# Chengyuann/AutoStyle-TTS

Hardware: AMD Instinct MI355X
Metric: synthesized audio sec/wall-sec (RTF^-1) + style-kNN QPS, IEMOCAP test batch (higher is better)
Workload: dtype f16; 1 GPU; BASELINE configs[1]: batch=8 utterances/GPU, kNN Q=8 x N=1000 x D=6144 k=3, synthesis Tt=32 Tp=150 Ts=250 (fixed-length decode, EOS ignored) -> 430 mel frames -> 110080 samples @ 22050 Hz; CosyVoice-300M shapes, random-init weights; parallelism=dp1 (model + bank replicated, utterances sharded, all-gather of style ids only)

## Files before the change

### autostyle-tts_amd/csrc/ops_audio.hip

```cpp
#include "common.h"
#include "toplist.h"
#include "xlane.h"

namespace astts {

static constexpr double kTwoPi = 6.283185307179586476925286766559;

__global__ __launch_bounds__(256) void f0_prefix(const float* __restrict__ f0, double* __restrict__ pre, int tm) {
    __shared__ double carry;
    __shared__ double buf[256];
    const int b = blockIdx.x, tid = threadIdx.x;
    if (tid == 0) carry = 0.0;
    __syncthreads();
    for (int base = 0; base < tm; base += 256) {
        const int i = base + tid;
        const double v = i < tm ? (double)f0[(int64_t)b * tm + i] : 0.0;
        buf[tid] = v;
        __syncthreads();
        for (int off = 1; off < 256; off <<= 1) {
            const double add = tid >= off ? buf[tid - off] : 0.0;
            __syncthreads();
            buf[tid] += add;
            __syncthreads();
        }
        if (i < tm) pre[(int64_t)b * tm + i] = carry + buf[tid] - v;
        __syncthreads();
        if (tid == 255) carry += buf[255];
        __syncthreads();
    }
}

struct NsfArgs {
    const float* f0;
    const double* pre;
    const float* phase0;
    const float* noise;
    const float* lin_w;
    const float* lin_b;
    float* out;
    int b, tm, up, nh;
    float sr, sine_amp, noise_std, voiced_thr;
};

__global__ __launch_bounds__(256) void nsf_source(NsfArgs a) {
    const int64_t L = (int64_t)a.tm * a.up;
    const int64_t total = (int64_t)a.b * L;
    for (int64_t i = (int64_t)blockIdx.x * 256 + threadIdx.x; i < total; i += (int64_t)gridDim.x * 256) {
        const int bb = (int)(i / L);
        const int64_t s = i - (int64_t)bb * L;
        const int f = (int)(s / a.up);
        const int r = (int)(s - (int64_t)f * a.up);
        const float f0 = a.f0[(int64_t)bb * a.tm + f];
        const double cum = (a.pre[(int64_t)bb * a.tm + f] * (double)a.up + (double)(r + 1) * (double)f0) / (double)a.sr;
        const float uv = f0 > a.voiced_thr ? 1.0f : 0.0f;
        const float namp = uv * a.noise_std + (1.0f - uv) * a.sine_amp / 3.0f;
        float acc = a.lin_b[0];
        for (int hI = 0; hI < a.nh; ++hI) {
            double ph = cum * (double)(hI + 1);
            ph -= floor(ph);
            const float theta = (float)(kTwoPi * ph);
            const float sine = a.sine_amp * sinf(theta + a.phase0[bb * a.nh + hI]);
            const float v = sine * uv + namp * a.noise[i * a.nh + hI];
            acc += a.lin_w[hI] * v;
        }
        a.out[i] = tanhf(acc);
    }
}

__device__ __forceinline__ float hann16(int n) {
    return 0.5f - 0.5f * cosf((float)(kTwoPi / 16.0) * (float)n);
}

__global__ __launch_bounds__(256) void stft16(const float* __restrict__ x, float* __restrict__ y, int b, int64_t Lmax, int64_t F,
                                              const int* __restrict__ lens) {
    const int64_t total = (int64_t)b * F;
    for (int64_t i = (int64_t)blockIdx.x * 256 + threadIdx.x; i < total; i += (int64_t)gridDim.x * 256) {
        const int bb = (int)(i / F);
        const int64_t f = i - (int64_t)bb * F;
        const float* xb = x + (int64_t)bb * Lmax;
        const int64_t L = lens ? min((int64_t)lens[bb], Lmax) : Lmax;
        float* o = y + i * 18;
        if (f > L / 4) {
#pragma unroll
            for (int k = 0; k < 18; ++k) o[k] = 0.0f;
            continue;
        }
        float w[16];
#pragma unroll
        for (int n = 0; n < 16; ++n) {
            int64_t s = 4 * f - 8 + n;
            if (s < 0) s = -s;
            if (s >= L) s = 2 * (L - 1) - s;
            w[n] = hann16(n) * xb[s];
        }
#pragma unroll
        for (int k = 0; k < 9; ++k) {
            float re = 0.0f, im = 0.0f;
#pragma unroll
            for (int n = 0; n < 16; ++n) {
                const int ph = (k * n) & 15;
                const float cs = cosf((float)(kTwoPi / 16.0) * (float)ph);
                const float sn = sinf((float)(kTwoPi / 16.0) * (float)ph);
                re += w[n] * cs;
                im -= w[n] * sn;
            }
            o[k] = re;
            o[9 + k] = im;
        }
    }
}

__global__ __launch_bounds__(256) void istft16(const float* __restrict__ y, float* __restrict__ wav, int b, int64_t Fmax,
                                               float mag_clip, float audio_limit, const int* __restrict__ frame_lens) {
    const int64_t L = 4 * (Fmax - 1);
    const int64_t total = (int64_t)b * L;
    for (int64_t i = (int64_t)blockIdx.x * 256 + threadIdx.x; i < total; i += (int64_t)gridDim.x * 256) {
        const int bb = (int)(i / L);
        const int64_t t = i - (int64_t)bb * L;
        const int64_t F = frame_lens ? min((int64_t)frame_lens[bb], Fmax) : Fmax;
        if (t >= 4 * (F - 1)) {
            wav[i] = 0.0f;
            continue;
        }
        const int64_t tp = t + 8;
        float num = 0.0f, den = 0.0f;
        const int64_t f_hi = tp / 4;
#pragma unroll
        for (int q = 0; q < 4; ++q) {
            const int64_t f = f_hi - q;
            const int n = (int)(tp - 4 * f);
            if (f < 0 || f >= F) continue;
            const float* fr = y + ((int64_t)bb * Fmax + f) * 18;
            float xs = 0.0f;
#pragma unroll
            for (int k = 0; k < 9; ++k) {
                const float mag = fminf(__expf(fr[k]), mag_clip);
                const float ph = sinf(fr[9 + k]);
                const float re = mag * cosf(ph), im = mag * sinf(ph);
                const int idx = (k * n) & 15;
                const float cs = cosf((float)(kTwoPi / 16.0) * (float)idx);
                const float sn = sinf((float)(kTwoPi / 16.0) * (float)idx);
                const float ck = (k == 0 || k == 8) ? 1.0f : 2.0f;
                xs += ck * (re * cs - ((k == 0 || k == 8) ? 0.0f : im * sn));
            }
            const float wn = hann16(n);
            num += wn * xs * (1.0f / 16.0f);
            den += wn * wn;
        }
        const float v = den > 1e-11f ? num / den : 0.0f;
        wav[i] = fminf(fmaxf(v, -audio_limit), audio_limit);
    }
}

struct SampleArgs {
    const float* logits;
    const int* history;
    const float* u;
    int* out;
    int* hist_w;
    const int* forced;
    int clamp_out;
    const int* eos_min_rows;
    int b, v, hist_len, hist_ld, top_k, win, eos, ignore_eos;
    float top_p, tau_r;
};

static constexpr int RS_NT = 1024;
__global__ __launch_bounds__(RS_NT) void ras_sample(const float* p_logits, const int* p_eos_min_rows, int p_v, int p_hist_len, int p_eos, int p_ignore_eos,
                                                    SampleArgs a_in) {
    __builtin_amdgcn_s_setprio(3);
    SampleArgs a = a_in;
    a.logits = p_logits; a.eos_min_rows = p_eos_min_rows; a.v = p_v; a.hist_len = p_hist_len; a.eos = p_eos; a.ignore_eos = p_ignore_eos;
    extern __shared__ float prob[];
    __shared__ float red_max[RS_NT / 64], red_sum[RS_NT / 64];
    __shared__ float sh_s[RS_NT];
    __shared__ int sh_i[RS_NT];
    __shared__ float s_bcast;
    __shared__ int s_tok;
    __shared__ unsigned hist[3][2048];
    __shared__ int s_sel_bin[3], s_sel_rem[3], s_cnt;
    const int bb = blockIdx.x, tid = threadIdx.x, lane = tid & 63, wid = tid >> 6;
    const float* lg = a.logits + (int64_t)bb * a.v;
    const bool eos_window = a.eos_min_rows ? (a.hist_len < a.eos_min_rows[bb]) : ((a.ignore_eos & 1) != 0);
    const bool reject = eos_window && (a.ignore_eos & 2) != 0;
    const bool mask_eos = eos_window && !reject;
    const int h0 = a.hist_len > a.win ? a.hist_len - a.win : 0;
    const bool win_in_wave = a.hist_len - h0 <= 64;
    float u_first = 0.0f, u_second = 0.0f;
    int hwin = -1;
    if (wid == 0) {
        u_first = a.u[bb * 2];
        u_second = a.u[bb * 2 + 1];
        if (win_in_wave && h0 + lane < a.hist_len) hwin = a.history[(int64_t)bb * a.hist_ld + h0 + lane];
    }
    for (int i = tid; i < 3 * 2048; i += RS_NT) (&hist[0][0])[i] = 0u;
    if (tid == 0) s_cnt = 0;
    if (tid < 16 && ((a.v + 15) & ~15) - 16 + tid >= a.v) prob[((a.v + 15) & ~15) - 16 + tid] = 0.0f;
    float mx = -INFINITY;
    for (int base = 0; base < a.v; base += 8 * RS_NT) {
        float xv[8];
#pragma unroll
        for (int u = 0; u < 8; ++u) xv[u] = lg[min(base + u * RS_NT + tid, a.v - 1)];
#pragma unroll
        for (int u = 0; u < 8; ++u) {
            const int i = base + u * RS_NT + tid;
            if (i < a.v) {
                float x = xv[u];
                if (mask_eos && i == a.eos) x = -INFINITY;
                prob[i] = x;
                mx = fmaxf(mx, x);
            }
        }
    }
    mx = xmax<1>(xmax<2>(xmax<4>(xmax<8>(xmax<16>(xmax<32>(mx))))));
    if (lane == 0) red_max[wid] = mx;
    __syncthreads();
    mx = red_max[0];
#pragma unroll
    for (int w = 1; w < RS_NT / 64; ++w) mx = fmaxf(mx, red_max[w]);
    float sum = 0.0f;
    for (int i = tid; i < a.v; i += RS_NT) {
        const float e = __expf(prob[i] - mx);
        prob[i] = e;
        sum += e;
    }
    sum = wave_sum_desc(sum);
    if (lane == 0) red_sum[wid] = sum;
    __syncthreads();
    float tot = 0.0f;
#pragma unroll
    for (int w = 0; w < RS_NT / 64; ++w) tot += red_sum[w];
    const float inv = 1.0f / tot;
    const int kk = a.top_k < 64 ? a.top_k : 64;
    TopList<float> tl;
    tl.init();
    unsigned prefix = 0u, known = 0u;
    {
        int remaining = kk < a.v ? kk : a.v;
#pragma unroll 1
        for (int pass = 0; pass < 3; ++pass) {
            const int shift = pass == 0 ? 21 : (pass == 1 ? 10 : 0);
            const int bins = pass == 2 ? 1024 : 2048;
            unsigned* h = hist[pass];
            for (int i = tid; i < a.v; i += RS_NT) {
                float pv = prob[i];
                if (pass == 0) {
                    pv *= inv;
                    prob[i] = pv;
                }
                const unsigned key = __float_as_uint(pv);
                if ((key & known) == prefix) atomicAdd(&h[(key >> shift) & (bins - 1)], 1u);
            }
            __syncthreads();
            if (wid == 0) {
                const int per = bins >> 6;
                unsigned hv[32];
#pragma unroll
                for (int j = 0; j < 32; ++j) hv[j] = j < per ? h[lane * per + j] : 0u;
                unsigned local = 0u;
#pragma unroll
                for (int j = 0; j < 32; ++j) local += hv[j];
                unsigned incl = local;
#pragma unroll
                for (int off = 1; off < 64; off <<= 1) {
                    const unsigned tv = __shfl_down(incl, off, 64);
                    if (lane + off < 64) incl += tv;
                }
                const unsigned above = incl - local;
                if (above < (unsigned)remaining && (unsigned)remaining <= incl) {
                    unsigned acc = above;
                    bool done = false;
#pragma unroll
                    for (int j = 31; j >= 0; --j) {
                        if (j < per && !done) {
                            if (acc + hv[j] >= (unsigned)remaining) {
                                s_sel_bin[pass] = lane * per + j;
                                s_sel_rem[pass] = remaining - (int)acc;
                                done = true;
                            } else {
                                acc += hv[j];
                            }
                        }
                    }
                }
            }
            __syncthreads();
            prefix |= (unsigned)s_sel_bin[pass] << shift;
            known |= (unsigned)(bins - 1) << shift;
            remaining = s_sel_rem[pass];
        }
        for (int i = tid; i < a.v; i += RS_NT) {
            if (__float_as_uint(prob[i]) >= prefix) {
                const int pos = atomicAdd(&s_cnt, 1);
                if (pos < 64) {
                    sh_s[pos] = prob[i];
                    sh_i[pos] = i;
                }
            }
        }
        __syncthreads();
    }
    const bool fast = s_cnt <= 64;
    if (fast) {
        if (wid == 0) tl.seed(sh_s[lane], sh_i[lane], lane < s_cnt, lane);
    } else {
        bool seeded = false;
        for (int base = wid * 64; base < a.v; base += RS_NT) {
            const int i = base + lane;
            const bool valid = i < a.v;
            const float pv = valid ? prob[i] : -INFINITY;
            if (!seeded) {
                tl.seed(pv, i, valid, lane);
                seeded = true;
            } else {
                tl.offer(pv, i, valid, lane, kk);
            }
        }
        __syncthreads();
        merge_lists<float>(tl, sh_s, sh_i, kk);
    }
    if (wid == 0) {
        sh_s[lane] = tl.s;
        sh_i[lane] = tl.idx;
        __builtin_amdgcn_s_waitcnt(0xc07f);
        __builtin_amdgcn_wave_barrier();
        float cum = 0.0f;
        int cnt = 0;
        bool open = true;
#pragma unroll 8
        for (int r = 0; r < kk; ++r) {
            const float pr = sh_s[r];
            const int ir = sh_i[r];
            open = open && ir != kNoIdx && cum < a.top_p && cnt < a.top_k;
            if (open) {
                cum += pr;
                ++cnt;
            }
        }
        auto repeated = [&](int t) -> bool {
            int rep = 0;
            if (win_in_wave) {
                rep = __popcll(__ballot(hwin == t));
            } else {
                for (int i0 = h0; i0 < a.hist_len; i0 += 64) {
                    const int i = i0 + lane;
                    const bool hit = i < a.hist_len && a.history[(int64_t)bb * a.hist_ld + i] == t;
                    rep += __popcll(__ballot(hit));
                }
            }
            return (float)rep >= (float)a.win * a.tau_r;
        };
        int tok;
        bool fallback;
        if (!reject) {
            const float target = u_first * cum;
            float run = 0.0f;
            tok = sh_i[cnt > 0 ? cnt - 1 : 0];
            bool found = false;
#pragma unroll 8
            for (int r = 0; r < kk; ++r) {
                const float pr = sh_s[r];
                const int ir = sh_i[r];
                if (r < cnt) {
                    run += pr;
                    if (!found && run > target) {
                        tok = ir;
                        found = true;
                    }
                }
            }
            fallback = repeated(tok);
        } else {
            const float p_eos = prob[a.eos];
            const float pr_l = lane < cnt ? sh_s[lane] : 0.0f;
            const int ir_l = lane < cnt ? sh_i[lane] : -1;
            int repc = 0;
            if (win_in_wave) {
                const int wl = a.hist_len - h0;
                for (int j = 0; j < wl; ++j) repc += __builtin_amdgcn_readlane(hwin, j) == ir_l ? 1 : 0;
            } else {
                for (int i = h0; i < a.hist_len; ++i) repc += a.history[(int64_t)bb * a.hist_ld + i] == ir_l ? 1 : 0;
            }
            const bool rep_l = (float)repc >= (float)a.win * a.tau_r;
            const unsigned long long direct = __ballot(lane < cnt && ir_l != a.eos && !rep_l);
            const unsigned long long again = __ballot(lane < cnt && ir_l != a.eos && rep_l);
            float asum = 0.0f, prep = 0.0f;
            for (int r = 0; r < cnt; ++r) {
                const float v = __builtin_bit_cast(float, __builtin_amdgcn_readlane(__builtin_bit_cast(int, pr_l), r));
                if (direct >> r & 1ull) asum += v;
                else if (again >> r & 1ull) prep += v;
            }
            const float target = u_first * (asum + prep * (1.0f - p_eos));
            float run = 0.0f;
            tok = -1;
            for (int r = 0; r < cnt && tok < 0; ++r) {
                if (direct >> r & 1ull) {
                    run += __builtin_bit_cast(float, __builtin_amdgcn_readlane(__builtin_bit_cast(int, pr_l), r));
                    if (run > target) tok = __builtin_amdgcn_readlane(ir_l, r);
                }
            }
            fallback = tok < 0;
        }
        if (lane == 0) {
            s_tok = tok;
            s_bcast = fallback ? 1.0f : 0.0f;
        }
    }
    __syncthreads();
    if (s_bcast > 0.5f && tid == 0) {
        const float p_skip = reject ? prob[a.eos] : 0.0f;
        if (reject) prob[a.eos] = 0.0f;
        const float target = reject ? u_second * (1.0f - p_skip) : u_second;
        float run = 0.0f;
        int tok = -1;
        const int vpad = (a.v + 15) & ~15;
        for (int base = 0; base < vpad && tok < 0; base += 16) {
            const float4 q0 = *reinterpret_cast<const float4*>(prob + base), q1 = *reinterpret_cast<const float4*>(prob + base + 4);
            const float4 q2 = *reinterpret_cast<const float4*>(prob + base + 8), q3 = *reinterpret_cast<const float4*>(prob + base + 12);
            const float pv[16] = {q0.x, q0.y, q0.z, q0.w, q1.x, q1.y, q1.z, q1.w, q2.x, q2.y, q2.z, q2.w, q3.x, q3.y, q3.z, q3.w};
            float r[16];
            r[0] = run + pv[0];
#pragma unroll
            for (int k = 1; k < 16; ++k) r[k] = r[k - 1] + pv[k];
            if (r[15] > target) {
#pragma unroll
                for (int k = 15; k >= 0; --k)
                    if (r[k] > target) tok = base + k;
            }
            run = r[15];
        }
        if (tok < 0 || tok >= a.v) {
            tok = 0;
            for (int i = a.v - 1; i > 0; --i)
                if (prob[i] > 0.0f) {
                    tok = i;
                    break;
                }
        }
        s_tok = tok;
    }
    __syncthreads();
    if (tid == 0) {
        int tok = s_tok;
        if (a.forced) tok = a.forced[(int64_t)bb * a.hist_ld + a.hist_len];
        if (a.hist_w) a.hist_w[(int64_t)bb * a.hist_ld + a.hist_len] = tok;
        a.out[bb] = (a.clamp_out >= 0 && tok > a.clamp_out) ? a.clamp_out : tok;
    }
}


__global__ __launch_bounds__(256) void resample_poly(const float* __restrict__ x, const float* __restrict__ kern, float* __restrict__ y,
                                                     int b, int64_t n_in, int64_t n_out, int up, int down, int width, int taps) {
    const int64_t total = (int64_t)b * n_out;
    for (int64_t i = (int64_t)blockIdx.x * 256 + threadIdx.x; i < total; i += (int64_t)gridDim.x * 256) {
        const int64_t bb = i / n_out, o = i - bb * n_out;
        const int64_t f = o / up;
        const int ph = (int)(o - f * up);
        const float* xr = x + bb * n_in;
        const float* kr = kern + (int64_t)ph * taps;
        const int64_t s0 = f * down - width;
        float acc = 0.0f;
        for (int j = 0; j < taps; ++j) {
            const int64_t s = s0 + j;
            const float kv = kr[j];
            if (kv != 0.0f && s >= 0 && s < n_in) acc = fmaf(kv, xr[s], acc);
        }
        y[i] = acc;
    }
}

enum { MEL_MATCHA = 0, MEL_WHISPER = 1, MEL_KALDI = 2 };
template <int MODE>
__global__ __launch_bounds__(256) void mel_frames(const float* __restrict__ wav, const float* __restrict__ window,
                                                  const float* __restrict__ fb, float* __restrict__ out, int64_t n, int frames,
                                                  int n_fft, int hop, int n_mels, float floor_, int* __restrict__ gmax, int frame_len,
                                                  float scale, float preemph) {
    constexpr bool WHISPER = MODE == MEL_WHISPER;
    constexpr bool KALDI = MODE == MEL_KALDI;
    extern __shared__ float sm[];
    float* fr = sm;
    float* twc = sm + n_fft;
    float* tws = twc + n_fft;
    float* mag = tws + n_fft;
    const int f = blockIdx.x, bb = blockIdx.y, tid = threadIdx.x;
    const int pad = WHISPER ? n_fft / 2 : (n_fft - hop) / 2;
    const float* w = wav + (int64_t)bb * n;
    int n_time = n_fft;
    if constexpr (KALDI) {
        __shared__ float s_part[4];
        n_time = frame_len;
        const float* src = w + (int64_t)f * hop;
        float part = 0.0f;
        for (int i = tid; i < n_fft; i += 256) {
            const float v = i < frame_len ? src[i] * scale : 0.0f;
            fr[i] = v;
            part += v;
            float sv, cv;
            sincospif(2.0f * (float)i / (float)n_fft, &sv, &cv);
            twc[i] = cv;
            tws[i] = sv;
        }
        for (int off = 32; off >= 1; off >>= 1) part += __shfl_xor(part, off, 64);
        if ((tid & 63) == 0) s_part[tid >> 6] = part;
        __syncthreads();
        const float mean = ((s_part[0] + s_part[1]) + (s_part[2] + s_part[3])) / (float)frame_len;
        float cur[2], prv[2];
#pragma unroll
        for (int j = 0; j < 2; ++j) {
            const int i = tid + 256 * j;
            cur[j] = i < frame_len ? fr[i] - mean : 0.0f;
            prv[j] = (i >= 1 && i < frame_len) ? fr[i - 1] - mean : 0.0f;
        }
        __syncthreads();
#pragma unroll
        for (int j = 0; j < 2; ++j) {
            const int i = tid + 256 * j;
            if (i < frame_len) fr[i] = (i == 0 ? cur[j] * (1.0f - preemph) : cur[j] - preemph * prv[j]) * window[i];
        }
    } else {
        for (int i = tid; i < n_fft; i += 256) {
            int64_t s = (int64_t)f * hop + i - pad;
            if (s < 0) s = -s;
            if (s >= n) s = 2 * (n - 1) - s;
            s = s < 0 ? 0 : (s >= n ? n - 1 : s);
            fr[i] = w[s] * window[i];
            float sv, cv;
            sincospif(2.0f * (float)i / (float)n_fft, &sv, &cv);
            twc[i] = cv;
            tws[i] = sv;
        }
    }
    __syncthreads();
    const int nb = n_fft / 2 + 1;
    for (int k = tid; k < nb; k += 256) {
        float re = 0.0f, im = 0.0f;
        int idx = 0;
        for (int i = 0; i < n_time; ++i) {
            re = fmaf(fr[i], twc[idx], re);
            im = fmaf(fr[i], tws[idx], im);
            idx += k;
            if (idx >= n_fft) idx -= n_fft;
        }
        mag[k] = (WHISPER || KALDI) ? re * re + im * im : sqrtf(re * re + im * im + 1e-9f);
    }
    __syncthreads();
    float vmax = -INFINITY;
    for (int m = tid; m < n_mels; m += 256) {
        const float* fr_ = fb + (int64_t)m * nb;
        float acc = 0.0f;
        for (int k = 0; k < nb; ++k) acc = fmaf(fr_[k], mag[k], acc);
        if constexpr (WHISPER) {
            const float v = log10f(fmaxf(acc, floor_));
            out[((int64_t)bb * n_mels + m) * frames + f] = v;
            vmax = fmaxf(vmax, v);
        } else {
            out[((int64_t)bb * frames + f) * n_mels + m] = logf(fmaxf(acc, floor_));
        }
    }
    if constexpr (WHISPER) {
        for (int off = 32; off >= 1; off >>= 1) vmax = fmaxf(vmax, __shfl_xor(vmax, off, 64));
        if ((tid & 63) == 0 && vmax > -INFINITY) {
            const int bits = __float_as_int(vmax);
            atomicMax(gmax + bb, bits >= 0 ? bits : (int)(0x80000000u - (unsigned)bits));
        }
    }
}

__global__ __launch_bounds__(256) void whisper_floor(float* __restrict__ x, const int* __restrict__ gmax, int64_t per_item, int64_t total) {
    for (int64_t i = (int64_t)blockIdx.x * 256 + threadIdx.x; i < total; i += (int64_t)gridDim.x * 256) {
        const int key = gmax[i / per_item];
        const float mx = __int_as_float(key >= 0 ? key : (int)(0x80000000u - (unsigned)key));
        x[i] = (fmaxf(x[i], mx - 8.0f) + 4.0f) * 0.25f;
    }
}

}

using namespace astts;

static inline int grid_for_a(int64_t total) {
    int64_t b = (total + 255) / 256;
    return (int)(b > 4096 ? 4096 : (b < 1 ? 1 : b));
}

extern "C" {

size_t astts_op_nsf_source_workspace_bytes(int32_t b, int32_t tm) { return (size_t)b * tm * sizeof(double); }

int astts_op_nsf_source(const float* f0, const float* phase0, const float* noise, const float* lin_w, const float* lin_b,
                        float* out, int32_t b, int32_t tm, int32_t upsample, int32_t n_harm_plus1, float sample_rate,
                        float sine_amp, float noise_std, float voiced_threshold, void* workspace, size_t workspace_bytes,
                        astts_stream_t stream) {
    ASTTS_REQUIRE(f0 && phase0 && noise && lin_w && lin_b && out && workspace, ASTTS_ERR_INVALID, "astts_op_nsf_source: null pointer");
    ASTTS_REQUIRE(b >= 1 && tm >= 1 && upsample >= 1 && n_harm_plus1 >= 1 && n_harm_plus1 <= 32, ASTTS_ERR_INVALID,
                  "astts_op_nsf_source: bad shape");
    ASTTS_REQUIRE(workspace_bytes >= astts_op_nsf_source_workspace_bytes(b, tm), ASTTS_ERR_WORKSPACE,
                  "astts_op_nsf_source: workspace too small");
    hipStream_t st = (hipStream_t)stream;
    hipLaunchKernelGGL(f0_prefix, dim3(b), dim3(256), 0, st, f0, (double*)workspace, tm);
    ASTTS_CHECK_LAUNCH();
    NsfArgs a{f0, (const double*)workspace, phase0, noise, lin_w, lin_b, out, b, tm, upsample, n_harm_plus1,
              sample_rate, sine_amp, noise_std, voiced_threshold};
    hipLaunchKernelGGL(nsf_source, dim3(grid_for_a((int64_t)b * tm * upsample)), dim3(256), 0, st, a);
    ASTTS_CHECK_LAUNCH();
    return ASTTS_OK;
}

int astts_op_stft16(const float* x, float* y, int32_t b, int64_t n_samples, const int32_t* lens, astts_stream_t stream) {
    ASTTS_REQUIRE(x && y && b >= 1 && n_samples >= 16 && n_samples % 4 == 0, ASTTS_ERR_INVALID, "astts_op_stft16: bad argument");
    const int64_t F = n_samples / 4 + 1;
    hipLaunchKernelGGL(stft16, dim3(grid_for_a((int64_t)b * F)), dim3(256), 0, (hipStream_t)stream, x, y, b, n_samples, F, lens);
    ASTTS_CHECK_LAUNCH();
    return ASTTS_OK;
}

int astts_op_istft16(const float* y, float* wav, int32_t b, int64_t frames, float mag_clip, float audio_limit, const int32_t* frame_lens,
                     astts_stream_t stream) {
    ASTTS_REQUIRE(y && wav && b >= 1 && frames >= 2, ASTTS_ERR_INVALID, "astts_op_istft16: bad argument");
    hipLaunchKernelGGL(istft16, dim3(grid_for_a((int64_t)b * 4 * (frames - 1))), dim3(256), 0, (hipStream_t)stream, y,
                       wav, b, frames, mag_clip, audio_limit, frame_lens);
    ASTTS_CHECK_LAUNCH();
    return ASTTS_OK;
}

int astts_op_ras_sample(const float* logits, const int32_t* history, const float* uniforms, int32_t* out_tokens,
                        int32_t b, int32_t vocab, int32_t hist_len, int32_t hist_ld, int32_t top_k, float top_p,
                        int32_t win_size, float tau_r, int32_t eos_id, int32_t ignore_eos, astts_stream_t stream) {
    ASTTS_REQUIRE(logits && uniforms && out_tokens && (history || hist_len == 0), ASTTS_ERR_INVALID, "astts_op_ras_sample: null pointer");
    ASTTS_REQUIRE(b >= 1 && vocab >= 2 && vocab <= 15000 && top_k >= 1 && top_k <= 64 && hist_len >= 0, ASTTS_ERR_INVALID,
                  "astts_op_ras_sample: bad shape b=%d vocab=%d top_k=%d", b, vocab, top_k);
    ASTTS_REQUIRE(!(ignore_eos & 2) || (eos_id >= 0 && eos_id < vocab), ASTTS_ERR_RANGE, "astts_op_ras_sample: eos_id=%d outside [0, %d) with the reject policy", eos_id, vocab);
    SampleArgs a{logits, history, uniforms, out_tokens, nullptr, nullptr, -1, nullptr, b, vocab, hist_len, hist_ld, top_k, win_size, eos_id, ignore_eos, top_p, tau_r};
    hipLaunchKernelGGL(ras_sample, dim3(b), dim3(RS_NT), (size_t)((vocab + 15) & ~15) * sizeof(float), (hipStream_t)stream, a.logits, a.eos_min_rows, a.v,
                       a.hist_len, a.eos, a.ignore_eos, a);
    ASTTS_CHECK_LAUNCH();
    return ASTTS_OK;
}

int astts_op_ras_sample_ex(const float* logits, int32_t* history, const float* uniforms, int32_t* out_tokens, int32_t b,
                           int32_t vocab, int32_t hist_len, int32_t hist_ld, int32_t top_k, float top_p, int32_t win_size,
                           float tau_r, int32_t eos_id, int32_t ignore_eos, const int32_t* eos_min_rows, const int32_t* forced,
                           astts_stream_t stream) {
    ASTTS_REQUIRE(logits && uniforms && out_tokens && history, ASTTS_ERR_INVALID, "astts_op_ras_sample_ex: null pointer");
    ASTTS_REQUIRE(b >= 1 && vocab >= 2 && vocab <= 15000 && top_k >= 1 && top_k <= 64 && hist_len >= 0 && hist_len < hist_ld,
                  ASTTS_ERR_INVALID, "astts_op_ras_sample_ex: bad shape b=%d vocab=%d top_k=%d hist_len=%d", b, vocab, top_k, hist_len);
    ASTTS_REQUIRE(!(ignore_eos & 2) || (eos_id >= 0 && eos_id < vocab), ASTTS_ERR_RANGE, "astts_op_ras_sample_ex: eos_id=%d outside [0, %d) with the reject policy", eos_id, vocab);
    SampleArgs a{logits, history, uniforms, out_tokens, history, forced, eos_id - 1, eos_min_rows, b, vocab, hist_len, hist_ld, top_k, win_size,
                 eos_id, ignore_eos, top_p, tau_r};
    hipLaunchKernelGGL(ras_sample, dim3(b), dim3(RS_NT), (size_t)((vocab + 15) & ~15) * sizeof(float), (hipStream_t)stream, a.logits, a.eos_min_rows, a.v,
                       a.hist_len, a.eos, a.ignore_eos, a);
    ASTTS_CHECK_LAUNCH();
    return ASTTS_OK;
}


int astts_op_resample_poly(const float* x, const float* kern, float* y, int32_t b, int64_t n_in, int64_t n_out, int32_t up, int32_t down,
                           int32_t width, astts_stream_t stream) {
    ASTTS_REQUIRE(x && kern && y, ASTTS_ERR_INVALID, "astts_op_resample_poly: null pointer");
    ASTTS_REQUIRE(b >= 1 && n_in >= 1 && n_out >= 1 && up >= 1 && down >= 1 && width >= 0, ASTTS_ERR_INVALID,
                  "astts_op_resample_poly: bad shape");
    hipLaunchKernelGGL(resample_poly, dim3(grid_for_a((int64_t)b * n_out)), dim3(256), 0, (hipStream_t)stream, x, kern, y, b, n_in, n_out, up,
                       down, width, 2 * width + down);
    ASTTS_CHECK_LAUNCH();
    return ASTTS_OK;
}

int astts_op_mel_spectrogram(const float* wav, const float* window, const float* mel_fb, float* out, int32_t b, int64_t n_samples,
                             int32_t n_fft, int32_t hop, int32_t n_mels, float log_floor, astts_stream_t stream) {
    ASTTS_REQUIRE(wav && window && mel_fb && out, ASTTS_ERR_INVALID, "astts_op_mel_spectrogram: null pointer");
    ASTTS_REQUIRE(b >= 1 && n_fft >= 16 && n_fft <= 2048 && hop >= 1 && hop <= n_fft && n_mels >= 1 && log_floor > 0.0f,
                  ASTTS_ERR_INVALID, "astts_op_mel_spectrogram: bad shape n_fft=%d hop=%d n_mels=%d", n_fft, hop, n_mels);
    const int pad = (n_fft - hop) / 2;
    ASTTS_REQUIRE(n_samples > pad, ASTTS_ERR_INVALID, "astts_op_mel_spectrogram: %lld samples are shorter than the reflect padding %d",
                  (long long)n_samples, pad);
    const int64_t frames = (n_samples + 2 * pad - n_fft) / hop + 1;
    ASTTS_REQUIRE(frames >= 1 && frames < (1 << 30), ASTTS_ERR_INVALID, "astts_op_mel_spectrogram: frames=%lld", (long long)frames);
    const size_t lds = sizeof(float) * ((size_t)3 * n_fft + n_fft / 2 + 1);
    hipLaunchKernelGGL(mel_frames<MEL_MATCHA>, dim3((unsigned)frames, (unsigned)b), dim3(256), lds, (hipStream_t)stream, wav, window, mel_fb, out,
                       n_samples, (int)frames, n_fft, hop, n_mels, log_floor, (int*)nullptr, n_fft, 1.0f, 0.0f);
    ASTTS_CHECK_LAUNCH();
    return ASTTS_OK;
}

int astts_op_kaldi_fbank(const float* wav, const float* window, const float* mel_fb, float* out, int32_t b, int64_t n_samples, int32_t frame_len,
                         int32_t hop, int32_t n_fft, int32_t n_mels, float scale, float preemph, float log_floor, astts_stream_t stream) {
    ASTTS_REQUIRE(wav && window && mel_fb && out, ASTTS_ERR_INVALID, "astts_op_kaldi_fbank: null pointer");
    ASTTS_REQUIRE(b >= 1 && frame_len >= 16 && frame_len <= n_fft && n_fft <= 512 && hop >= 1 && n_mels >= 1 && log_floor > 0.0f, ASTTS_ERR_INVALID,
                  "astts_op_kaldi_fbank: bad shape frame_len=%d n_fft=%d hop=%d n_mels=%d (one thread holds two samples of a frame: n_fft <= 512)",
                  frame_len, n_fft, hop, n_mels);
    ASTTS_REQUIRE(n_samples >= frame_len, ASTTS_ERR_INVALID, "astts_op_kaldi_fbank: %lld samples are shorter than one frame of %d",
                  (long long)n_samples, frame_len);
    const int64_t frames = 1 + (n_samples - frame_len) / hop;
    ASTTS_REQUIRE(frames < (1 << 30), ASTTS_ERR_INVALID, "astts_op_kaldi_fbank: frames=%lld", (long long)frames);
    const size_t lds = sizeof(float) * ((size_t)3 * n_fft + n_fft / 2 + 1);
    hipLaunchKernelGGL(mel_frames<MEL_KALDI>, dim3((unsigned)frames, (unsigned)b), dim3(256), lds, (hipStream_t)stream, wav, window, mel_fb, out,
                       n_samples, (int)frames, n_fft, hop, n_mels, log_floor, (int*)nullptr, frame_len, scale, preemph);
    ASTTS_CHECK_LAUNCH();
    return ASTTS_OK;
}

size_t astts_op_whisper_log_mel_workspace_bytes(int32_t b) { return (size_t)(b > 0 ? b : 0) * sizeof(int); }

int astts_op_whisper_log_mel(const float* wav, const float* window, const float* mel_fb, float* out, int32_t b, int64_t n_samples,
                             int32_t n_fft, int32_t hop, int32_t n_mels, void* workspace, size_t workspace_bytes, astts_stream_t stream) {
    ASTTS_REQUIRE(wav && window && mel_fb && out && workspace, ASTTS_ERR_INVALID, "astts_op_whisper_log_mel: null pointer");
    ASTTS_REQUIRE(b >= 1 && n_fft >= 16 && n_fft <= 2048 && hop >= 1 && hop <= n_fft && n_mels >= 1, ASTTS_ERR_INVALID,
                  "astts_op_whisper_log_mel: bad shape n_fft=%d hop=%d n_mels=%d", n_fft, hop, n_mels);
    ASTTS_REQUIRE(workspace_bytes >= astts_op_whisper_log_mel_workspace_bytes(b), ASTTS_ERR_WORKSPACE, "astts_op_whisper_log_mel: workspace too small");
    ASTTS_REQUIRE(n_samples > n_fft / 2, ASTTS_ERR_INVALID, "astts_op_whisper_log_mel: %lld samples are shorter than the reflect padding %d",
                  (long long)n_samples, n_fft / 2);
    const int64_t frames = n_samples / hop;
    ASTTS_REQUIRE(frames >= 1 && frames < (1 << 30), ASTTS_ERR_INVALID, "astts_op_whisper_log_mel: frames=%lld", (long long)frames);
    hipStream_t st = (hipStream_t)stream;
    ASTTS_CHECK_HIP(hipMemsetD32Async((hipDeviceptr_t)workspace, (int)0x80000000u, (size_t)b, st));
    const size_t lds = sizeof(float) * ((size_t)3 * n_fft + n_fft / 2 + 1);
    hipLaunchKernelGGL(mel_frames<MEL_WHISPER>, dim3((unsigned)frames, (unsigned)b), dim3(256), lds, st, wav, window, mel_fb, out, n_samples, (int)frames,
                       n_fft, hop, n_mels, 1e-10f, (int*)workspace, n_fft, 1.0f, 0.0f);
    ASTTS_CHECK_LAUNCH();
    const int64_t total = (int64_t)b * n_mels * frames;
    hipLaunchKernelGGL(whisper_floor, dim3(grid_for_a(total)), dim3(256), 0, st, out, (const int*)workspace, (int64_t)n_mels * frames, total);
    ASTTS_CHECK_LAUNCH();
    return ASTTS_OK;
}

}
```

### autostyle-tts_amd/csrc/toplist.h

```cpp
#pragma once
#include "common.h"
#include "xlane.h"

namespace astts {

static constexpr int kNoIdx = 0x7fffffff;

template <typename T>
__device__ __forceinline__ bool better(T sa, int ia, T sb, int ib) {
    return (sa > sb) || (sa == sb && ia < ib);
}

template <typename T>
struct TopList {
    T s;
    int idx;
    __device__ __forceinline__ void init() {
        s = -INFINITY;
        idx = kNoIdx;
    }
    __device__ __forceinline__ void sort_desc(int lane) {
#pragma unroll
        for (int k = 2; k <= 64; k <<= 1) {
#pragma unroll
            for (int j = k >> 1; j > 0; j >>= 1) {
                T os = lane_xor_dyn(s, j);
                int oi = lane_xor_dyn(idx, j);
                const bool up = (lane & k) == 0;
                const bool lower = (lane & j) == 0;
                const bool other_better = better<T>(os, oi, s, idx);
                const bool take = (up == lower) ? other_better : !other_better;
                if (take) {
                    s = os;
                    idx = oi;
                }
            }
        }
    }
    __device__ __forceinline__ void insert(T xs, int xi, int lane, int c) {
        const bool mine_better = better<T>(s, idx, xs, xi) && lane < c;
        const int pos = __popcll(__ballot(mine_better));
        T ups = __shfl_up(s, 1, 64);
        int upi = __shfl_up(idx, 1, 64);
        if (lane == pos) {
            s = xs;
            idx = xi;
        } else if (lane > pos) {
            s = ups;
            idx = upi;
        }
    }
    __device__ __forceinline__ void offer(T vs, int vi, bool valid, int lane, int c) {
        T ws = __shfl(s, c - 1, 64);
        int wi = __shfl(idx, c - 1, 64);
        unsigned long long mask = __ballot(valid && better<T>(vs, vi, ws, wi));
        while (mask) {
            const int src = __ffsll((long long)mask) - 1;
            mask &= mask - 1;
            T xs = __shfl(vs, src, 64);
            int xi = __shfl(vi, src, 64);
            insert(xs, xi, lane, c);
        }
    }
    __device__ __forceinline__ void seed(T vs, int vi, bool valid, int lane) {
        s = valid ? vs : (T)-INFINITY;
        idx = valid ? vi : kNoIdx;
        sort_desc(lane);
    }
};

template <typename T>
__device__ __forceinline__ void merge_lists(TopList<T>& tl, T* sh_s, int* sh_i, int c) {
    const int tid = threadIdx.x, lane = tid & 63, wid = tid >> 6;
    const int nw = blockDim.x >> 6;
    sh_s[wid * 64 + lane] = tl.s;
    sh_i[wid * 64 + lane] = tl.idx;
    __syncthreads();
    if (wid == 0) {
        for (int w = 1; w < nw; ++w) {
            T v = sh_s[w * 64 + lane];
            int vi = sh_i[w * 64 + lane];
            tl.offer(v, vi, lane < c && vi != kNoIdx, lane, c);
        }
    }
}


}
```

Baseline: 478.3 audio-s/wall-s.

## Add register-resident top-k sampling kernel with threshold pruning for RAS decode

Adds a new ras_sample_regs kernel that keeps logits in registers across 512 threads, computes the softmax in registers, and prunes candidates per wave using a bitonic-sorted per-lane-max threshold, so only a small candidate set is merged into the top-k list. The old 1024-thread kernel is kept behind an env flag, and shared draw, walk and emit logic is factored into helpers. The goal is to cut LDS traffic and the long offer/merge loops of the per-step sampling kernel in autoregressive decode. If pruning yields more than 64 candidates it falls back to a full scan, and the larger register arrays risk lower occupancy.

```diff
diff --git a/autostyle-tts_amd/csrc/ops_audio.hip b/autostyle-tts_amd/csrc/ops_audio.hip
--- a/autostyle-tts_amd/csrc/ops_audio.hip
+++ b/autostyle-tts_amd/csrc/ops_audio.hip
@@ -164,6 +164,132 @@
     int b, v, hist_len, hist_ld, top_k, win, eos, ignore_eos;
     float top_p, tau_r;
 };
+
+__device__ __forceinline__ void rs_draw(const SampleArgs& a, int bb, int lane, const TopList<float>& tl, float* sh_s, int* sh_i, const float* prob,
+                                        int kk, bool reject, float u_first, int hwin, int h0, bool win_in_wave, int& tok_out, bool& fallback_out) {
+    sh_s[lane] = tl.s;
+    sh_i[lane] = tl.idx;
+    __builtin_amdgcn_s_waitcnt(0xc07f);
+    __builtin_amdgcn_wave_barrier();
+    float cum = 0.0f;
+    int cnt = 0;
+    bool open = true;
+#pragma unroll 8
+    for (int r = 0; r < kk; ++r) {
+        const float pr = sh_s[r];
+        const int ir = sh_i[r];
+        open = open && ir != kNoIdx && cum < a.top_p && cnt < a.top_k;
+        if (open) {
+            cum += pr;
+            ++cnt;
+        }
+    }
+    auto repeated = [&](int t) -> bool {
+        int rep = 0;
+        if (win_in_wave) {
+            rep = __popcll(__ballot(hwin == t));
+        } else {
+            for (int i0 = h0; i0 < a.hist_len; i0 += 64) {
+                const int i = i0 + lane;
+                const bool hit = i < a.hist_len && a.history[(int64_t)bb * a.hist_ld + i] == t;
+                rep += __popcll(__ballot(hit));
+            }
+        }
+        return (float)rep >= (float)a.win * a.tau_r;
+    };
+    int tok;
+    bool fallback;
+    if (!reject) {
+        const float target = u_first * cum;
+        float run = 0.0f;
+        tok = sh_i[cnt > 0 ? cnt - 1 : 0];
+        bool found = false;
+#pragma unroll 8
+        for (int r = 0; r < kk; ++r) {
+            const float pr = sh_s[r];
+            const int ir = sh_i[r];
+            if (r < cnt) {
+                run += pr;
+                if (!found && run > target) {
+                    tok = ir;
+                    found = true;
+                }
+            }
+        }
+        fallback = repeated(tok);
+    } else {
+        const float p_eos = prob[a.eos];
+        const float pr_l = lane < cnt ? sh_s[lane] : 0.0f;
+        const int ir_l = lane < cnt ? sh_i[lane] : -1;
+        int repc = 0;
+        if (win_in_wave) {
+            const int wl = a.hist_len - h0;
+            for (int j = 0; j < wl; ++j) repc += __builtin_amdgcn_readlane(hwin, j) == ir_l ? 1 : 0;
+        } else {
+            for (int i = h0; i < a.hist_len; ++i) repc += a.history[(int64_t)bb * a.hist_ld + i] == ir_l ? 1 : 0;
+        }
+        const bool rep_l = (float)repc >= (float)a.win * a.tau_r;
+        const unsigned long long direct = __ballot(lane < cnt && ir_l != a.eos && !rep_l);
+        const unsigned long long again = __ballot(lane < cnt && ir_l != a.eos && rep_l);
+        float asum = 0.0f, prep = 0.0f;
+        for (int r = 0; r < cnt; ++r) {
+            const float v = __builtin_bit_cast(float, __builtin_amdgcn_readlane(__builtin_bit_cast(int, pr_l), r));
+            if (direct >> r & 1ull) asum += v;
+            else if (again >> r & 1ull) prep += v;
+        }
+        const float target = u_first * (asum + prep * (1.0f - p_eos));
+        float run = 0.0f;
+        tok = -1;
+        for (int r = 0; r < cnt && tok < 0; ++r) {
+            if (direct >> r & 1ull) {
+                run += __builtin_bit_cast(float, __builtin_amdgcn_readlane(__builtin_bit_cast(int, pr_l), r));
+                if (run > target) tok = __builtin_amdgcn_readlane(ir_l, r);
+            }
+        }
+        fallback = tok < 0;
+    }
+    tok_out = tok;
+    fallback_out = fallback;
+}
+
+__device__ __forceinline__ int rs_walk(const SampleArgs& a, float* prob, bool reject, float u_second) {
+    const float p_skip = reject ? prob[a.eos] : 0.0f;
+    if (reject) prob[a.eos] = 0.0f;
+    const float target = reject ? u_second * (1.0f - p_skip) : u_second;
+    float run = 0.0f;
+    int tok = -1;
+    const int vpad = (a.v + 15) & ~15;
+    for (int base = 0; base < vpad && tok < 0; base += 16) {
+        const float4 q0 = *reinterpret_cast<const float4*>(prob + base), q1 = *reinterpret_cast<const float4*>(prob + base + 4);
+        const float4 q2 = *reinterpret_cast<const float4*>(prob + base + 8), q3 = *reinterpret_cast<const float4*>(prob + base + 12);
+        const float pv[16] = {q0.x, q0.y, q0.z, q0.w, q1.x, q1.y, q1.z, q1.w, q2.x, q2.y, q2.z, q2.w, q3.x, q3.y, q3.z, q3.w};
+        float r[16];
+        r[0] = run + pv[0];
+#pragma unroll
+        for (int k = 1; k < 16; ++k) r[k] = r[k - 1] + pv[k];
+        if (r[15] > target) {
+#pragma unroll
+            for (int k = 15; k >= 0; --k)
+                if (r[k] > target) tok = base + k;
+        }
+        run = r[15];
+    }
+    if (tok < 0 || tok >= a.v) {
+        tok = 0;
+        for (int i = a.v - 1; i > 0; --i)
+            if (prob[i] > 0.0f) {
+                tok = i;
+                break;
+            }
+    }
+    return tok;
+}
+
+__device__ __forceinline__ void rs_emit(const SampleArgs& a, int bb, int tok) {
+    if (a.forced) tok = a.forced[(int64_t)bb * a.hist_ld + a.hist_len];
+    if (a.hist_w) a.hist_w[(int64_t)bb * a.hist_ld + a.hist_len] = tok;
+    a.out[bb] = (a.clamp_out >= 0 && tok > a.clamp_out) ? a.clamp_out : tok;
+}
 
 static constexpr int RS_NT = 1024;
 __global__ __launch_bounds__(RS_NT) void ras_sample(const float* p_logits, const int* p_eos_min_rows, int p_v, int p_hist_len, int p_eos, int p_ignore_eos,
@@ -320,132 +446,169 @@
         merge_lists<float>(tl, sh_s, sh_i, kk);
     }
     if (wid == 0) {
-        sh_s[lane] = tl.s;
-        sh_i[lane] = tl.idx;
-        __builtin_amdgcn_s_waitcnt(0xc07f);
-        __builtin_amdgcn_wave_barrier();
-        float cum = 0.0f;
-        int cnt = 0;
-        bool open = true;
-#pragma unroll 8
-        for (int r = 0; r < kk; ++r) {
-            const float pr = sh_s[r];
-            const int ir = sh_i[r];
-            open = open && ir != kNoIdx && cum < a.top_p && cnt < a.top_k;
-            if (open) {
-                cum += pr;
-                ++cnt;
-            }
-        }
-        auto repeated = [&](int t) -> bool {
-            int rep = 0;
-            if (win_in_wave) {
-                rep = __popcll(__ballot(hwin == t));
-            } else {
-                for (int i0 = h0; i0 < a.hist_len; i0 += 64) {
-                    const int i = i0 + lane;
-                    const bool hit = i < a.hist_len && a.history[(int64_t)bb * a.hist_ld + i] == t;
-                    rep += __popcll(__ballot(hit));
-                }
-            }
-            return (float)rep >= (float)a.win * a.tau_r;
-        };
         int tok;
         bool fallback;
-        if (!reject) {
-            const float target = u_first * cum;
-            float run = 0.0f;
-            tok = sh_i[cnt > 0 ? cnt - 1 : 0];
-            bool found = false;
-#pragma unroll 8
-            for (int r = 0; r < kk; ++r) {
-                const float pr = sh_s[r];
-                const int ir = sh_i[r];
-                if (r < cnt) {
-                    run += pr;
-                    if (!found && run > target) {
-                        tok = ir;
-                        found = true;
-                    }
-                }
-            }
-            fallback = repeated(tok);
-        } else {
-            const float p_eos = prob[a.eos];
-            const float pr_l = lane < cnt ? sh_s[lane] : 0.0f;
-            const int ir_l = lane < cnt ? sh_i[lane] : -1;
-            int repc = 0;
-            if (win_in_wave) {
-                const int wl = a.hist_len - h0;
-                for (int j = 0; j < wl; ++j) repc += __builtin_amdgcn_readlane(hwin, j) == ir_l ? 1 : 0;
-            } else {
-                for (int i = h0; i < a.hist_len; ++i) repc += a.history[(int64_t)bb * a.hist_ld + i] == ir_l ? 1 : 0;
-            }
-            const bool rep_l = (float)repc >= (float)a.win * a.tau_r;
-            const unsigned long long direct = __ballot(lane < cnt && ir_l != a.eos && !rep_l);
-            const unsigned long long again = __ballot(lane < cnt && ir_l != a.eos && rep_l);
-            float asum = 0.0f, prep = 0.0f;
-            for (int r = 0; r < cnt; ++r) {
-                const float v = __builtin_bit_cast(float, __builtin_amdgcn_readlane(__builtin_bit_cast(int, pr_l), r));
-                if (direct >> r & 1ull) asum += v;
-                else if (again >> r & 1ull) prep += v;
-            }
-            const float target = u_first * (asum + prep * (1.0f - p_eos));
-            float run = 0.0f;
-            tok = -1;
-            for (int r = 0; r < cnt && tok < 0; ++r) {
-                if (direct >> r & 1ull) {
-                    run += __builtin_bit_cast(float, __builtin_amdgcn_readlane(__builtin_bit_cast(int, pr_l), r));
-                    if (run > target) tok = __builtin_amdgcn_readlane(ir_l, r);
-                }
-            }
-            fallback = tok < 0;
-        }
+        rs_draw(a, bb, lane, tl, sh_s, sh_i, prob, kk, reject, u_first, hwin, h0, win_in_wave, tok, fallback);
         if (lane == 0) {
             s_tok = tok;
             s_bcast = fallback ? 1.0f : 0.0f;
         }
     }
     __syncthreads();
-    if (s_bcast > 0.5f && tid == 0) {
-        const float p_skip = reject ? prob[a.eos] : 0.0f;
-        if (reject) prob[a.eos] = 0.0f;
-        const float target = reject ? u_second * (1.0f - p_skip) : u_second;
-        float run = 0.0f;
-        int tok = -1;
-        const int vpad = (a.v + 15) & ~15;
-        for (int base = 0; base < vpad && tok < 0; base += 16) {
-            const float4 q0 = *reinterpret_cast<const float4*>(prob + base), q1 = *reinterpret_cast<const float4*>(prob + base + 4);
-            const float4 q2 = *reinterpret_cast<const float4*>(prob + base + 8), q3 = *reinterpret_cast<const float4*>(prob + base + 12);
-            const float pv[16] = {q0.x, q0.y, q0.z, q0.w, q1.x, q1.y, q1.z, q1.w, q2.x, q2.y, q2.z, q2.w, q3.x, q3.y, q3.z, q3.w};
-            float r[16];
-            r[0] = run + pv[0];
-#pragma unroll
-            for (int k = 1; k < 16; ++k) r[k] = r[k - 1] + pv[k];
-            if (r[15] > target) {
-#pragma unroll
-                for (int k = 15; k >= 0; --k)
-                    if (r[k] > target) tok = base + k;
-            }
-            run = r[15];
-        }
-        if (tok < 0 || tok >= a.v) {
-            tok = 0;
-            for (int i = a.v - 1; i > 0; --i)
-                if (prob[i] > 0.0f) {
-                    tok = i;
-                    break;
-                }
-        }
-        s_tok = tok;
-    }
-    __syncthreads();
-    if (tid == 0) {
-        int tok = s_tok;
-        if (a.forced) tok = a.forced[(int64_t)bb * a.hist_ld + a.hist_len];
-        if (a.hist_w) a.hist_w[(int64_t)bb * a.hist_ld + a.hist_len] = tok;
-        a.out[bb] = (a.clamp_out >= 0 && tok > a.clamp_out) ? a.clamp_out : tok;
-    }
+    if (s_bcast > 0.5f && tid == 0) s_tok = rs_walk(a, prob, reject, u_second);
+    __syncthreads();
+    if (tid == 0) rs_emit(a, bb, s_tok);
+}
+
+template <int NS>
+__device__ __forceinline__ int rs_prune(const float (&s)[NS], const int (&id)[NS], int lane, int kk, float* dst_s, int* dst_i) {
+    float lm = s[0];
+#pragma unroll
+    for (int n = 1; n < NS; ++n) lm = fmaxf(lm, s[n]);
+    const float sorted = sort_desc_keys(lm, lane);
+    const float t = fmaxf(__builtin_bit_cast(float, __builtin_amdgcn_readlane(__builtin_bit_cast(int, sorted), kk - 1)), 0.0f);
+    int base = 0;
+#pragma unroll
+    for (int n = 0; n < NS; ++n) {
+        const bool hit = s[n] >= t;
+        const unsigned long long m = __ballot(hit);
+        const int pos = base + (int)__builtin_amdgcn_mbcnt_hi((unsigned)(m >> 32), __builtin_amdgcn_mbcnt_lo((unsigned)m, 0u));
+        if (hit && pos < 64) {
+            dst_s[pos] = s[n];
+            dst_i[pos] = id[n];
+        }
+        base += __popcll(m);
+    }
+    return base;
+}
+
+static constexpr int RR_NT = 512, RR_NW = RR_NT / 64;
+template <int NV>
+__global__ __launch_bounds__(RR_NT) void ras_sample_regs(const float* p_logits, const int* p_eos_min_rows, int p_v, int p_hist_len, int p_eos,
+                                                         int p_ignore_eos, SampleArgs a_in) {
+    __builtin_amdgcn_s_setprio(3);
+    SampleArgs a = a_in;
+    a.logits = p_logits; a.eos_min_rows = p_eos_min_rows; a.v = p_v; a.hist_len = p_hist_len; a.eos = p_eos; a.ignore_eos = p_ignore_eos;
+    extern __shared__ float prob[];
+    __shared__ float red_max[RR_NW], red_sum[2 * RR_NW];
+    __shared__ float cand_s[RR_NW][64];
+    __shared__ int cand_i[RR_NW][64];
+    __shared__ int cand_n[RR_NW];
+    __shared__ float sh_s[64];
+    __shared__ int sh_i[64];
+    const int bb = blockIdx.x, tid = threadIdx.x, lane = tid & 63, wid = tid >> 6;
+    const float* lg = a.logits + (int64_t)bb * a.v;
+    float x[NV];
+#pragma unroll
+    for (int n = 0; n < NV; ++n) x[n] = lg[min(n * RR_NT + tid, a.v - 1)];
+    const int h0 = a.hist_len > a.win ? a.hist_len - a.win : 0;
+    const bool win_in_wave = a.hist_len - h0 <= 64;
+    float u_first = 0.0f, u_second = 0.0f;
+    int hwin = -1;
+    if (wid == 0) {
+        u_first = a.u[bb * 2];
+        u_second = a.u[bb * 2 + 1];
+        if (win_in_wave && h0 + lane < a.hist_len) hwin = a.history[(int64_t)bb * a.hist_ld + h0 + lane];
+    }
+    const bool eos_window = a.eos_min_rows ? (a.hist_len < a.eos_min_rows[bb]) : ((a.ignore_eos & 1) != 0);
+    const bool reject = eos_window && (a.ignore_eos & 2) != 0;
+    const bool mask_eos = eos_window && !reject;
+    if (tid < 16 && ((a.v + 15) & ~15) - 16 + tid >= a.v) prob[((a.v + 15) & ~15) - 16 + tid] = 0.0f;
+    float mx = -INFINITY;
+#pragma unroll
+    for (int n = 0; n < NV; ++n) {
+        const int i = n * RR_NT + tid;
+        if (i >= a.v || (mask_eos && i == a.eos)) x[n] = -INFINITY;
+        mx = fmaxf(mx, x[n]);
+    }
+    mx = xmax<1>(xmax<2>(xmax<4>(xmax<8>(xmax<16>(xmax<32>(mx))))));
+    if (lane == 0) red_max[wid] = mx;
+    __syncthreads();
+    mx = red_max[0];
+#pragma unroll
+    for (int w = 1; w < RR_NW; ++w) mx = fmaxf(mx, red_max[w]);
+    float p[NV];
+    float acc[2] = {0.0f, 0.0f};
+#pragma unroll
+    for (int n = 0; n < NV; ++n) {
+        p[n] = __expf(x[n] - mx);
+        acc[n & 1] += p[n];
+    }
+    const float s_even = wave_sum_desc(acc[0]), s_odd = wave_sum_desc(acc[1]);
+    if (lane == 0) {
+        red_sum[wid] = s_even;
+        red_sum[wid + RR_NW] = s_odd;
+    }
+    __syncthreads();
+    float tot = 0.0f;
+#pragma unroll
+    for (int w = 0; w < 2 * RR_NW; ++w) tot += red_sum[w];
+    const float inv = 1.0f / tot;
+    int id[NV];
+#pragma unroll
+    for (int n = 0; n < NV; ++n) {
+        id[n] = n * RR_NT + tid;
+        p[n] *= inv;
+        if (id[n] < a.v) prob[id[n]] = p[n];
+        else p[n] = -1.0f;
+    }
+    const int kk = a.top_k < 64 ? a.top_k : 64;
+    const int mine = rs_prune<NV>(p, id, lane, kk, cand_s[wid], cand_i[wid]);
+    if (lane == 0) cand_n[wid] = mine;
+    __syncthreads();
+    if (wid != 0) return;
+    float q[RR_NW];
+    int qi[RR_NW];
+    int rot = 0;
+    bool general = false;
+#pragma unroll
+    for (int w = 0; w < RR_NW; ++w) {
+        const int cn = __builtin_amdgcn_readfirstlane(cand_n[w]);
+        general = general || cn > 64;
+        const int j = (lane - rot) & 63;
+        q[w] = j < cn ? cand_s[w][j] : -1.0f;
+        qi[w] = cand_i[w][j];
+        rot += cn;
+    }
+    int left = 0;
+    if (!general) {
+        left = rs_prune<RR_NW>(q, qi, lane, kk, sh_s, sh_i);
+        general = left > 64;
+    }
+    TopList<float> tl;
+    tl.init();
+    if (!general) {
+        __builtin_amdgcn_s_waitcnt(0xc07f);
+        __builtin_amdgcn_wave_barrier();
+        tl.seed(sh_s[lane], sh_i[lane], lane < left, lane);
+    } else {
+        for (int base = 0; base < a.v; base += 64) {
+            const int i = base + lane;
+            const bool valid = i < a.v;
+            const float pv = valid ? prob[i] : -INFINITY;
+            if (base == 0) tl.seed(pv, i, valid, lane);
+            else tl.offer(pv, i, valid, lane, kk);
+        }
+    }
+    int tok;
+    bool fallback;
+    rs_draw(a, bb, lane, tl, sh_s, sh_i, prob, kk, reject, u_first, hwin, h0, win_in_wave, tok, fallback);
+    if (lane == 0) {
+        if (fallback) tok = rs_walk(a, prob, reject, u_second);
+        rs_emit(a, bb, tok);
+    }
+}
+
+static void launch_ras_sample(const SampleArgs& a, hipStream_t st) {
+    const size_t lds = (size_t)((a.v + 15) & ~15) * sizeof(float);
+    if (exp_env_int("ASTTS_RAS_RADIX", 0) != 0)
+        hipLaunchKernelGGL(ras_sample, dim3(a.b), dim3(RS_NT), lds, st, a.logits, a.eos_min_rows, a.v, a.hist_len, a.eos, a.ignore_eos, a);
+    else if (a.v <= 9 * RR_NT)
+        hipLaunchKernelGGL(ras_sample_regs<9>, dim3(a.b), dim3(RR_NT), lds, st, a.logits, a.eos_min_rows, a.v, a.hist_len, a.eos, a.ignore_eos, a);
+    else if (a.v <= 16 * RR_NT)
+        hipLaunchKernelGGL(ras_sample_regs<16>, dim3(a.b), dim3(RR_NT), lds, st, a.logits, a.eos_min_rows, a.v, a.hist_len, a.eos, a.ignore_eos, a);
+    else
+        hipLaunchKernelGGL(ras_sample_regs<30>, dim3(a.b), dim3(RR_NT), lds, st, a.logits, a.eos_min_rows, a.v, a.hist_len, a.eos, a.ignore_eos, a);
 }
 
 
@@ -631,8 +794,7 @@
                   "astts_op_ras_sample: bad shape b=%d vocab=%d top_k=%d", b, vocab, top_k);
     ASTTS_REQUIRE(!(ignore_eos & 2) || (eos_id >= 0 && eos_id < vocab), ASTTS_ERR_RANGE, "astts_op_ras_sample: eos_id=%d outside [0, %d) with the reject policy", eos_id, vocab);
     SampleArgs a{logits, history, uniforms, out_tokens, nullptr, nullptr, -1, nullptr, b, vocab, hist_len, hist_ld, top_k, win_size, eos_id, ignore_eos, top_p, tau_r};
-    hipLaunchKernelGGL(ras_sample, dim3(b), dim3(RS_NT), (size_t)((vocab + 15) & ~15) * sizeof(float), (hipStream_t)stream, a.logits, a.eos_min_rows, a.v,
-                       a.hist_len, a.eos, a.ignore_eos, a);
+    launch_ras_sample(a, (hipStream_t)stream);
     ASTTS_CHECK_LAUNCH();
     return ASTTS_OK;
 }
@@ -647,8 +809,7 @@
     ASTTS_REQUIRE(!(ignore_eos & 2) || (eos_id >= 0 && eos_id < vocab), ASTTS_ERR_RANGE, "astts_op_ras_sample_ex: eos_id=%d outside [0, %d) with the reject policy", eos_id, vocab);
     SampleArgs a{logits, history, uniforms, out_tokens, history, forced, eos_id - 1, eos_min_rows, b, vocab, hist_len, hist_ld, top_k, win_size,
                  eos_id, ignore_eos, top_p, tau_r};
-    hipLaunchKernelGGL(ras_sample, dim3(b), dim3(RS_NT), (size_t)((vocab + 15) & ~15) * sizeof(float), (hipStream_t)stream, a.logits, a.eos_min_rows, a.v,
-                       a.hist_len, a.eos, a.ignore_eos, a);
+    launch_ras_sample(a, (hipStream_t)stream);
     ASTTS_CHECK_LAUNCH();
     return ASTTS_OK;
 }
diff --git a/autostyle-tts_amd/csrc/toplist.h b/autostyle-tts_amd/csrc/toplist.h
--- a/autostyle-tts_amd/csrc/toplist.h
+++ b/autostyle-tts_amd/csrc/toplist.h
@@ -9,6 +9,18 @@
 template <typename T>
 __device__ __forceinline__ bool better(T sa, int ia, T sb, int ib) {
     return (sa > sb) || (sa == sb && ia < ib);
+}
+
+__device__ __forceinline__ float sort_desc_keys(float v, int lane) {
+#pragma unroll
+    for (int k = 2; k <= 64; k <<= 1) {
+#pragma unroll
+        for (int j = k >> 1; j > 0; j >>= 1) {
+            const float o = lane_xor_dyn(v, j);
+            v = (((lane & k) == 0) == ((lane & j) == 0)) ? fmaxf(v, o) : fminf(v, o);
+        }
+    }
+    return v;
 }
 
 template <typename T>
```

Measured after the change: 480.2 audio-s/wall-s, median of 5. About the same (+0.4%).
